# Nahuel-M/StereoVisionArray

Measured on AMD Instinct MI355X. Metric: Mdisparities/sec (W·H·D/s) at 1080p D=128, higher is better.
Workload: dtype u16

## Files before the change

stereovisionarray_amd/csrc/sva_tuning.h:

```cpp
#pragma once

#include <cstddef>

namespace sva {
namespace tune {

constexpr int kPfH4 = 40, kPfV4 = 24;
constexpr int kPfH8 = 32, kPfV8 = 12;
constexpr int kPfH12 = 24, kPfV12 = 8;
constexpr int kPfH16 = 12, kPfV16 = 8;
constexpr int kCLoadAux = 0;
constexpr int kCkptStoreAux = 0;
constexpr int kStaticCkptHitsMaxDpl = 4;

constexpr int kDiagPair4 = 0, kDiagPair8 = 1, kDiagPair12 = 0, kDiagPair16 = 0;
constexpr long long kDiagPairMinPixels = 1450000;
constexpr int kPathMinima4 = 0, kPathMinima8 = 1, kPathMinima12 = 0, kPathMinima16 = 0;
constexpr int kWtahvPfVolPair = 4;
constexpr int kWtahvTileLog2 = 3;
constexpr int kWtahvTileLog2Wide = 3;
constexpr int kWtahvPfVol = 3;
constexpr int kWtahvPfVol4 = 4;
constexpr int kWtahvPfVol16 = 2;
constexpr int kWtahvPinRowMin = 1;
constexpr int kWtahvPinWta = 1;
constexpr int kWtahvMinWaves = 1;

constexpr int kBatchMaxPairs = 8;
constexpr int kBatchCostStreams = 3;
constexpr int kBatchSubFrames = 4;
constexpr size_t kBatchMaxBytes = (size_t)24 << 30;

constexpr int kPlacementTrials = 6;
constexpr size_t kPlacementMinBytes = (size_t)4 << 30;

constexpr int kCensusRows = 16;
constexpr int kCensusCostMinD = 64;
constexpr int kCensusCostRows = 8;
constexpr int kCensusCostRowsSmall = 4;
constexpr int kCensusCostMinGroups = 1536;
constexpr int kCensusCostPx4 = 64, kCensusCostPx8 = 64, kCensusCostPx12 = 64, kCensusCostPx16 = 128;
constexpr int kCostStoreNT = 1;
constexpr int kCensusCostSlotOrder = 1;
constexpr int kCensusCost2Lines = 8;

constexpr int kPlaneOuKB = 24;
constexpr int kPlaneWords = 1024;
constexpr int kPlaneMinBlocks = 3;
constexpr int kPlaneStageMajor = 2;
constexpr int kPlaneNoHoistDiv = 0;
constexpr int kPlanePoLds = 1;
constexpr int kPlaneSplitMin = 3;
constexpr int kPlaneSplitMax = 6;
constexpr int kPlaneSplitRounds = 4;
constexpr int kPlaneSplitInner = 2;
constexpr int kPlaneWalkRange = 1;

}
}
```

stereovisionarray_amd/csrc/wta_hv.hip:

```cpp
#include "sgm_common.h"
#include "wta_common.h"
#include "sva_tuning.h"

namespace sva {
namespace {

using namespace sgm;

constexpr int TB = 256;
constexpr int TW = 16;

struct WtaHvGeom {
    int W, H, D, P1, P2, dmin;
    int ntx, nty;
    int nsx;
    int dreal;
    unsigned vol;
    unsigned hck;
    unsigned vck;
    int tiles;
};

template <int DPL, bool PAIR> constexpr int pf_vol() {
    return PAIR ? tune::kWtahvPfVolPair : DPL >= 16 ? tune::kWtahvPfVol16 : DPL <= 4 ? tune::kWtahvPfVol4 : tune::kWtahvPfVol;
}

#define SVA_WTAHV_CONF 0
#include "wta_hv_tile.inc"
#undef SVA_WTAHV_CONF
#define SVA_WTAHV_CONF 1
#include "wta_hv_tile.inc"
#undef SVA_WTAHV_CONF

template <int DPL, int TYL, bool PAIR, bool MN>
void wtahv_launch_mn(bool pad, dim3 grid, hipStream_t s, hipEvent_t start, hipEvent_t stop,
                     const uint8_t* C, const uint8_t* L4, const uint8_t* CK, const uint8_t* CKV,
                     const uint8_t* MNP, const WtaHvGeom& g, uint16_t* disp, float* sub,
                     const ConfOut* cf) {
    if (cf) {
        if (pad)
            hipExtLaunchKernelGGL((wta_hv_conf_kernel<DPL, TYL, true, PAIR, MN>), grid, dim3(TB), 0,
                                  s, start, stop, 0, C, L4, CK, CKV, MNP, g, disp, sub, *cf);
        else
            hipExtLaunchKernelGGL((wta_hv_conf_kernel<DPL, TYL, false, PAIR, MN>), grid, dim3(TB), 0,
                                  s, start, stop, 0, C, L4, CK, CKV, MNP, g, disp, sub, *cf);
        return;
    }
    if (pad)
        hipExtLaunchKernelGGL((wta_hv_kernel<DPL, TYL, true, PAIR, MN>), grid, dim3(TB), 0, s, start,
                              stop, 0, C, L4, CK, CKV, MNP, g, disp, sub);
    else
        hipExtLaunchKernelGGL((wta_hv_kernel<DPL, TYL, false, PAIR, MN>), grid, dim3(TB), 0, s, start,
                              stop, 0, C, L4, CK, CKV, MNP, g, disp, sub);
}
template <int DPL, int TYL, bool PAIR, bool MNEN>
void wtahv_launch(bool pad, dim3 grid, hipStream_t s, hipEvent_t start, hipEvent_t stop,
                  const uint8_t* C, const uint8_t* L4, const uint8_t* CK, const uint8_t* CKV,
                  const uint8_t* MNP, const WtaHvGeom& g, uint16_t* disp, float* sub,
                  const ConfOut* cf) {
    if constexpr (MNEN) {
        if (MNP) {
            wtahv_launch_mn<DPL, TYL, PAIR, true>(pad, grid, s, start, stop, C, L4, CK, CKV, MNP, g,
                                                  disp, sub, cf);
            return;
        }
    }
    wtahv_launch_mn<DPL, TYL, PAIR, false>(pad, grid, s, start, stop, C, L4, CK, CKV, nullptr, g,
                                           disp, sub, cf);
}

}

bool wta_hv_supported(int D) { return D == 64 || D == 128 || D == 192 || D == 256; }

hipError_t launch_wta_hv(Ctx& c, const uint8_t* C, const uint8_t* L4, const uint8_t* CK,
                         const uint8_t* CKV, int W, int H, int D, int P1, int P2, int dmin,
                         uint16_t* disp, float* sub, int dreal, int npair, bool pair,
                         const uint8_t* MN, const ConfOut* cf) {
    DispatchTimer t(c, "wta_hv");
    if (!wta_hv_supported(D)) return hipErrorInvalidValue;
    const TileGeom tg = tile_geom(W, H, D);
    WtaHvGeom g;
    g.W = W; g.H = H; g.D = D; g.P1 = P1; g.P2 = P2; g.dmin = dmin;
    g.dreal = dreal > 0 && dreal < D ? dreal : D;
    g.ntx = tg.ntx;
    g.nty = tg.nty;
    g.nsx = tg.nsx;
    const size_t vol = (size_t)W * H * D;
    if (vol >= (size_t)1 << 32) return hipErrorInvalidValue;
    g.vol = (unsigned)vol;
    g.hck = (unsigned)(tg.hck_bytes / 2);
    g.vck = (unsigned)(tg.vck_bytes / 2);
    const bool pad = g.dreal < D;
    if (npair < 1) return hipErrorInvalidValue;
    if (cf && (cf->uniqueness < 0 || cf->uniqueness > 100)) return hipErrorInvalidValue;
    g.tiles = g.ntx * g.nty;
    const dim3 grid((unsigned)(g.tiles * npair));
#define SVA_WTAHV(DPL_, TYL_, MN_)                                                            \
    wtahv_launch<DPL_, TYL_, false, (MN_) != 0>(pad, grid, c.stream, t.start, t.stop, C, L4,  \
                                                CK, CKV, MN, g, disp, sub, cf);               \
    t.used = true
#define SVA_WTAHV_P(DPL_, TYL_, EN_, MN_)                                                     \
    if (pair) {                                                                               \
        wtahv_launch<DPL_, TYL_, (EN_) != 0, (MN_) != 0>(pad, grid, c.stream, t.start,        \
                                                         t.stop, C, L4, CK, CKV, MN, g, disp, \
                                                         sub, cf);                            \
        t.used = true;                                                                        \
    } else {                                                                                  \
        SVA_WTAHV(DPL_, TYL_, MN_);                                                           \
    }
    constexpr int TYL = tune::kWtahvTileLog2, TYLW = tune::kWtahvTileLog2Wide;
    if (tg.seg_log2 != (D <= 128 ? TYL : TYLW)) return hipErrorInvalidValue;
    if (pair && (npair != 1 || !diag_pair_ok(D, P2))) return hipErrorInvalidValue;
    if (MN && (npair != 1 || !path_minima_enabled(D) || (1 << tg.seg_log2) != sgm::kMinimaSeg))
        return hipErrorInvalidValue;
    switch (D) {
        case 64: SVA_WTAHV_P(4, TYL, tune::kDiagPair4, tune::kPathMinima4); break;
        case 128: SVA_WTAHV_P(8, TYL, tune::kDiagPair8, tune::kPathMinima8); break;
        case 192: SVA_WTAHV_P(12, TYLW, tune::kDiagPair12, tune::kPathMinima12); break;
        case 256: SVA_WTAHV_P(16, TYLW, tune::kDiagPair16, tune::kPathMinima16); break;
        default: return hipErrorInvalidValue;
    }
#undef SVA_WTAHV_P
#undef SVA_WTAHV
    return hipGetLastError();
}

}
```

stereovisionarray_amd/csrc/wta_hv_tile.inc:

```
template <int DPL, int TYL, bool PAD, bool PAIR, bool MN>
#if SVA_WTAHV_CONF
__global__ __launch_bounds__(TB, tune::kWtahvMinWaves) void wta_hv_conf_kernel(
    const uint8_t* __restrict__ C, const uint8_t* __restrict__ L4, const uint8_t* __restrict__ CK,
    const uint8_t* __restrict__ CKV, const uint8_t* __restrict__ MNP, WtaHvGeom g,
    uint16_t* __restrict__ disp, float* __restrict__ sub, ConfOut cf) {
#else
__global__ __launch_bounds__(TB, tune::kWtahvMinWaves) void wta_hv_kernel(const uint8_t* __restrict__ C,
                                                    const uint8_t* __restrict__ L4,
                                                    const uint8_t* __restrict__ CK,
                                                    const uint8_t* __restrict__ CKV,
                                                    const uint8_t* __restrict__ MNP, WtaHvGeom g,
                                                    uint16_t* __restrict__ disp,
                                                    float* __restrict__ sub) {
#endif
    constexpr int NW = DPL / 4, NP = DPL / 2;
    constexpr int TY = 1 << TYL;
    constexpr int kPfVol = pf_vol<DPL, PAIR>();
    constexpr bool PIN = tune::kWtahvPinRowMin != 0;

    constexpr int SPR = TW / TY;
    static_assert(TY <= TW && TW % TY == 0, "tile rows must divide 16");
    const unsigned f = blockIdx.x / (unsigned)g.tiles;
    const unsigned tb = blockIdx.x - f * (unsigned)g.tiles;
    const int tx = (int)(tb % (unsigned)g.ntx);
    const int ty = (int)(tb / (unsigned)g.ntx);
    constexpr int NV = PAIR ? 2 : 4;
    static_assert(!MN || TY == kMinimaSeg, "path minima: 8-pixel segments");
    C += (size_t)f * g.vol;
    L4 += (size_t)f * NV * g.vol;
    CK += (size_t)f * 2 * g.hck;
    CKV += (size_t)f * 2 * g.vck;
    disp += (size_t)f * (size_t)g.W * (size_t)g.H;
    if (sub) sub += (size_t)f * (size_t)g.W * (size_t)g.H;
#if SVA_WTAHV_CONF
    if (cf.cost_min) cf.cost_min += (size_t)f * (size_t)g.W * (size_t)g.H;
    if (cf.cost_second) cf.cost_second += (size_t)f * (size_t)g.W * (size_t)g.H;
#endif
    const int slot = (int)(threadIdx.x >> 4);
    const int k = (int)(threadIdx.x & 15);
    const int W = g.W, H = g.H;
    const unsigned uD = (unsigned)g.D, uW = (unsigned)W;
    const unsigned P1 = (unsigned)g.P1, P2 = (unsigned)g.P2;
    const int x0 = tx * TW, y0 = ty * TY;
    const int nx = W - x0 < TW ? W - x0 : TW;
    const int ny = H - y0 < TY ? H - y0 : TY;
    const unsigned lane_d = (unsigned)(k * DPL);
    const rsrc_t rC = make_rsrc(C, g.vol);
    unsigned padm[NP];
#pragma unroll
    for (int j = 0; j < NP; j++) {
        const int dl = k * DPL + pair_d<DPL>(j, 0), dh = k * DPL + pair_d<DPL>(j, 1);
        padm[j] = PAD ? ((dl >= g.dreal ? 0x0000ffffu : 0u) | (dh >= g.dreal ? 0xffff0000u : 0u))
                      : 0u;
    }

    __shared__ unsigned vsum[TY * TW * 16 * NP];
    const int vb0 = k * NP, vb1 = k * NP + 4;
    auto vw = [&](int p) -> int { return (p < 4 ? vb0 : vb1) + (p & 3); };

    const bool vcol = slot < nx;
    const int hr = slot / SPR, hseg = slot % SPR;
    const int hx = x0 + hseg * TY;
    const int nh = W - hx < TY ? W - hx : TY;
    const bool hrow = hr < ny && nh > 0;
    const unsigned xv = (unsigned)(x0 + slot), yh = (unsigned)(y0 + hr);

    Words<NW> cv[TY], ch[TY];
#pragma unroll
    for (int r = 0; r < TY; r++)
        cv[r] = bload<NW>(rC, ((unsigned)(y0 + r) * uW + xv) * uD + lane_d);
    auto load_row = [&]() {
#pragma unroll
        for (int j = 0; j < TY; j++)
            ch[j] = bload<NW>(rC, (yh * uW + (unsigned)(hx + j)) * uD + lane_d);
    };
    load_row();
    Words<2> mv[2] = {}, mh[2] = {};
    if constexpr (MN) {
        const unsigned hmn = (unsigned)H * (unsigned)g.nsx * (unsigned)kMinimaSeg;
        const unsigned vmn = (unsigned)g.nty * uW * (unsigned)kMinimaSeg;
        const unsigned vo = ((unsigned)ty * uW + xv) * (unsigned)kMinimaSeg;
        const unsigned ho = ((unsigned)(y0 + (slot / SPR)) * (unsigned)g.nsx +
                             (unsigned)((x0 + (slot % SPR) * TY) >> TYL)) * (unsigned)kMinimaSeg;
#pragma unroll
        for (int d = 0; d < 2; d++) {
            mv[d] = bload<2>(make_rsrc(MNP + 2 * (size_t)hmn + (size_t)d * vmn, vmn), vo);
            mh[d] = bload<2>(make_rsrc(MNP + (size_t)d * hmn, hmn), ho);
        }
    }
    auto given_m = [](unsigned& m, const Words<2>& w, int i) {
        if constexpr (MN) m = minima_byte(w, i);
    };

    auto zero_state = [](unsigned (&A)[NP], unsigned& m) {
#pragma unroll
        for (int j = 0; j < NP; j++) A[j] = 0u;
        m = 0u;
    };
    unsigned Aa[NP], Ab[NP], ma, mb;
    Edges ea, eb;
    if (vcol) {
        if (ty > 0)
            load_state<DPL, PAD, PIN, MN>(make_rsrc(CKV, g.vck), ((unsigned)(ty - 1) * uW + xv) * uD + lane_d,
                                 Aa, ma, padm);
        else
            zero_state(Aa, ma);
        if (y0 + TY < H)
            load_state<DPL, PAD, PIN, MN>(make_rsrc(CKV + g.vck, g.vck),
                                 ((unsigned)(ty + 1) * uW + xv) * uD + lane_d, Ab, mb, padm);
        else
            zero_state(Ab, mb);
        auto keep = [&](unsigned (&dst)[NP], const unsigned (&A)[NP]) {
#pragma unroll
            for (int q = 0; q < NP; q++) dst[q] = A[q];
        };
        auto put_v = [&](int r, const unsigned (&ld)[NP], const unsigned (&Au)[NP],
                         const unsigned (&cw)[NW]) {
            unsigned V[NP];
#pragma unroll
            for (int p = 0; p < NP; p++) V[p] = ld[p] + Au[p];
            if constexpr (PAIR) {
                unsigned c4[NP];
                words_to_pairs<DPL>(cw, c4);
#pragma unroll
                for (int p = 0; p < NP; p++) V[p] += c4[p] << 2;
            }
            unsigned* dst = &vsum[(r * TW + slot) * 16 * NP];
#pragma unroll
            for (int p = 0; p < NP; p++) dst[vw(p)] = V[p];
        };
        unsigned LD[TY][NP];
        for_seq<TY>([&](auto I) {
            constexpr int i = decltype(I)::value;
            unsigned ow[NW];
            if (i < ny) {
                given_m(ma, mv[0], i);
                sgm_step<DPL, PIN, MN>(cv[i].w, Aa, ma, ow, P1, P2, ea);
                keep(LD[i], Aa);
            }
        });
        for_seq<TY>([&](auto Q) {
            constexpr int r = TY - 1 - decltype(Q)::value;
            if (r < ny) {
                unsigned lu[NW];
                given_m(mb, mv[1], TY - 1 - r);
                sgm_step<DPL, PIN, MN>(cv[r].w, Ab, mb, lu, P1, P2, eb);
                put_v(r, LD[r], Ab, cv[r].w);
            }
        });
    }
    const int hs = hx >> TYL;
    const unsigned ckrow = yh * (unsigned)g.nsx;
    Words<NW> ckw[2];
    rsrc_t rV[NV];
#pragma unroll
    for (int r = 0; r < NV; r++) rV[r] = make_rsrc(L4 + (size_t)r * g.vol, g.vol);
    Words<NW> rv[kPfVol][NV];
    auto issue = [&](int s, int j) {
        const unsigned off = (yh * uW + (unsigned)(hx + j)) * uD + lane_d;
#pragma unroll
        for (int r = 0; r < NV; r++) rv[s][r] = bload<NW, 2>(rV[r], off);
    };
    auto issue_first = [&]() {
        ckw[0] = bload<NW>(make_rsrc(CK, g.hck), (ckrow + (unsigned)(hs - 1)) * uD + lane_d);
        ckw[1] = bload<NW>(make_rsrc(CK + g.hck, g.hck), (ckrow + (unsigned)(hs + 1)) * uD + lane_d);
#pragma unroll
        for (int q = 0; q < kPfVol && q < TY; q++) issue(q, TY - 1 - q);
    };
    if (hrow) issue_first();
    __syncthreads();

    if (!hrow) return;
    if (hs > 0) state_from_words<DPL, PAD, PIN, MN>(ckw[0], Aa, ma, padm);
    else zero_state(Aa, ma);
    unsigned LF[TY][NP];
    for_seq<TY>([&](auto I) {
        constexpr int i = decltype(I)::value;
        unsigned ow[NW];
        if (i < nh) {
            given_m(ma, mh[0], i);
            sgm_step<DPL, PIN, MN>(ch[i].w, Aa, ma, ow, P1, P2, ea);
#pragma unroll
            for (int q = 0; q < NP; q++) LF[i][q] = Aa[q];
        }
    });
    if (hx + TY < W) state_from_words<DPL, PAD, PIN, MN>(ckw[1], Aa, ma, padm);
    else zero_state(Aa, ma);
    unsigned dres = 0u, sm = 0u, s0 = 0u;
#if SVA_WTAHV_CONF
    unsigned s2 = 0xffffu;
#endif
    const bool want_sub = sub != nullptr;
    unsigned dpair[NP];
#pragma unroll
    for (int j = 0; j < NP; j++)
        dpair[j] = (lane_d + (unsigned)pair_d<DPL>(j, 0)) | ((lane_d + (unsigned)pair_d<DPL>(j, 1)) << 16);
    unsigned* const vrow = &vsum[(hr * TW + hseg * TY) * 16 * NP];
    for_seq<TY>([&](auto Q) {
        constexpr int q = decltype(Q)::value, j = TY - 1 - q, s = q % kPfVol;
        if (j < nh) {
            unsigned ow[NW];
            given_m(ma, mh[1], q);
            sgm_step<DPL, PIN, MN>(ch[j].w, Aa, ma, ow, P1, P2, ea);
            unsigned* const vpix = vrow + j * 16 * NP;
            unsigned S[NP];
#pragma unroll
            for (int p = 0; p < NP; p++) S[p] = vpix[vw(p)] + Aa[p];
#pragma unroll
            for (int p = 0; p < NP; p++) S[p] += LF[j][p];
#pragma unroll
            for (int r = 0; r < NV; r++) unpack_add<NW>(rv[s][r].w, S);
            if constexpr (PAD) {
#pragma unroll
                for (int p = 0; p < NP; p++) S[p] |= padm[p];
            }
            const unsigned best = wta_pick_key_perm<DPL, PIN && tune::kWtahvPinWta>(S, dpair);
            const int ds = (int)(best & 0xffffu);
            if (want_sub) {
#pragma unroll
                for (int p = 0; p < NP; p++) vpix[vw(p)] = S[p];
            }
            dres = k == j ? (unsigned)ds : dres;
            s0 = k == j ? best >> 16 : s0;
#if SVA_WTAHV_CONF
            const unsigned sec = wta_second_key_perm<DPL, PIN && tune::kWtahvPinWta>(
                S, dpair, (unsigned)ds, lane_d);
            s2 = k == j ? sec : s2;
#endif
        }
        if constexpr (q + kPfVol < TY) {
            __builtin_amdgcn_sched_barrier(0);
            issue(s, TY - 1 - (q + kPfVol));
            __builtin_amdgcn_sched_barrier(0);
        }
    });
    if (want_sub) {
        __builtin_amdgcn_fence(__ATOMIC_RELEASE, "wavefront");
        __builtin_amdgcn_wave_barrier();
        __builtin_amdgcn_fence(__ATOMIC_ACQUIRE, "wavefront");
        if (k < nh) {
            const uint16_t* s16 = reinterpret_cast<const uint16_t*>(vrow + k * 16 * NP);
            const int ds = (int)dres;
            const int dm = ds > 0 ? ds - 1 : 0, dp = ds + 1 < 16 * DPL ? ds + 1 : ds;
            auto at = [&](int d) {
                const int kk = d / DPL, pp = pair_of<DPL>(d % DPL), hh = half_of<DPL>(d % DPL);
                return (unsigned)s16[2 * (kk * NP + pp) + hh];
            };
            sm = at(dm) | (at(dp) << 16);
        }
    }
    if (k < nh) {
        const size_t at = (size_t)yh * (size_t)W + (size_t)(hx + k);
#if SVA_WTAHV_CONF
        if (cf.cost_min) cf.cost_min[at] = (uint16_t)s0;
        if (cf.cost_second) cf.cost_second[at] = (uint16_t)s2;
        const bool rej = conf_reject(s0, s2, cf.uniqueness);
        disp[at] = rej ? (uint16_t)cf.invalid : (uint16_t)(g.dmin + (int)dres);
        if (want_sub) {
            const float v = subpixel(g.dmin, (int)dres, g.dreal, sm & 0xffffu, s0, sm >> 16);
            sub[at] = rej ? __builtin_nanf("") : v;
        }
#else
        disp[at] = (uint16_t)(g.dmin + (int)dres);
        if (want_sub) sub[at] = subpixel(g.dmin, (int)dres, g.dreal, sm & 0xffffu, s0, sm >> 16);
#endif
    }
}
```

Baseline: 335,600.

## Split WTA-HV tile start to overlap horizontal loads with vertical SGM pass

For the pair+minima variant, the horizontal-row cost loads, minima loads, horizontal checkpoint loads and the first volume prefetches are deferred. They are now issued between the forward and backward vertical SGM sweeps rather than upfront. The vertical checkpoint loads are issued together before being decoded. The aim is to cut register pressure and overlap global-memory latency with vertical-pass compute. The risk is that the loads land later, leaving less slack before the horizontal pass, and that the changed live ranges alter the register count.

Result: no change. 338,900, median of 6 (+1.0%).

```diff
diff --git a/stereovisionarray_amd/csrc/sva_tuning.h b/stereovisionarray_amd/csrc/sva_tuning.h
--- a/stereovisionarray_amd/csrc/sva_tuning.h
+++ b/stereovisionarray_amd/csrc/sva_tuning.h
@@ -17,6 +17,8 @@
 constexpr long long kDiagPairMinPixels = 1450000;
 constexpr int kPathMinima4 = 0, kPathMinima8 = 1, kPathMinima12 = 0, kPathMinima16 = 0;
 constexpr int kWtahvPfVolPair = 4;
+constexpr int kWtahvSplitStart = 1;
+constexpr int kWtahvPfVolPairEarly = 4;
 constexpr int kWtahvTileLog2 = 3;
 constexpr int kWtahvTileLog2Wide = 3;
 constexpr int kWtahvPfVol = 3;
diff --git a/stereovisionarray_amd/csrc/wta_hv.hip b/stereovisionarray_amd/csrc/wta_hv.hip
--- a/stereovisionarray_amd/csrc/wta_hv.hip
+++ b/stereovisionarray_amd/csrc/wta_hv.hip
@@ -23,6 +23,10 @@
 
 template <int DPL, bool PAIR> constexpr int pf_vol() {
     return PAIR ? tune::kWtahvPfVolPair : DPL >= 16 ? tune::kWtahvPfVol16 : DPL <= 4 ? tune::kWtahvPfVol4 : tune::kWtahvPfVol;
+}
+
+template <bool PAIR, int PF> constexpr int pf_vol_early() {
+    return !PAIR ? 0 : tune::kWtahvPfVolPairEarly < PF ? tune::kWtahvPfVolPairEarly : PF;
 }
 
 #define SVA_WTAHV_CONF 0
diff --git a/stereovisionarray_amd/csrc/wta_hv_tile.inc b/stereovisionarray_amd/csrc/wta_hv_tile.inc
--- a/stereovisionarray_amd/csrc/wta_hv_tile.inc
+++ b/stereovisionarray_amd/csrc/wta_hv_tile.inc
@@ -17,6 +17,8 @@
     constexpr int TY = 1 << TYL;
     constexpr int kPfVol = pf_vol<DPL, PAIR>();
     constexpr bool PIN = tune::kWtahvPinRowMin != 0;
+    constexpr bool SO = MN && PAIR && tune::kWtahvSplitStart != 0;
+    constexpr int kPfEarly = SO ? pf_vol_early<PAIR, kPfVol < TY ? kPfVol : TY>() : 0;
 
     constexpr int SPR = TW / TY;
     static_assert(TY <= TW && TW % TY == 0, "tile rows must divide 16");
@@ -74,7 +76,7 @@
         for (int j = 0; j < TY; j++)
             ch[j] = bload<NW>(rC, (yh * uW + (unsigned)(hx + j)) * uD + lane_d);
     };
-    load_row();
+    if constexpr (!SO) load_row();
     Words<2> mv[2] = {}, mh[2] = {};
     if constexpr (MN) {
         const unsigned hmn = (unsigned)H * (unsigned)g.nsx * (unsigned)kMinimaSeg;
@@ -85,7 +87,7 @@
 #pragma unroll
         for (int d = 0; d < 2; d++) {
             mv[d] = bload<2>(make_rsrc(MNP + 2 * (size_t)hmn + (size_t)d * vmn, vmn), vo);
-            mh[d] = bload<2>(make_rsrc(MNP + (size_t)d * hmn, hmn), ho);
+            if constexpr (!SO) mh[d] = bload<2>(make_rsrc(MNP + (size_t)d * hmn, hmn), ho);
         }
     }
     auto given_m = [](unsigned& m, const Words<2>& w, int i) {
@@ -96,10 +98,50 @@
 #pragma unroll
         for (int j = 0; j < NP; j++) A[j] = 0u;
         m = 0u;
+    };
+    Words<NW> rv[kPfVol][NV];
+    auto issue_early = [&]() {
+        if constexpr (kPfEarly > 0) {
+            if (hrow) {
+#pragma unroll
+                for (int q = 0; q < kPfEarly; q++) {
+                    const unsigned off = (yh * uW + (unsigned)(hx + TY - 1 - q)) * uD + lane_d;
+#pragma unroll
+                    for (int r = 0; r < NV; r++)
+                        rv[q][r] = bload<NW, 2>(make_rsrc(L4 + (size_t)r * g.vol, g.vol), off);
+                }
+            }
+        }
+    };
+    Words<NW> ckw[2];
+    auto load_h = [&]() {
+        load_row();
+        const unsigned hmn = (unsigned)H * (unsigned)g.nsx * (unsigned)kMinimaSeg;
+        const unsigned hseg0 = yh * (unsigned)g.nsx + (unsigned)(hx >> TYL);
+#pragma unroll
+        for (int d = 0; d < 2; d++)
+            mh[d] = bload<2>(make_rsrc(MNP + (size_t)d * hmn, hmn), hseg0 * (unsigned)kMinimaSeg);
+        if (hrow) {
+            ckw[0] = bload<NW>(make_rsrc(CK, g.hck), (hseg0 - 1u) * uD + lane_d);
+            ckw[1] = bload<NW>(make_rsrc(CK + g.hck, g.hck), (hseg0 + 1u) * uD + lane_d);
+        }
+        issue_early();
     };
     unsigned Aa[NP], Ab[NP], ma, mb;
     Edges ea, eb;
     if (vcol) {
+        if constexpr (SO) {
+            Words<NW> wa = {}, wb = {};
+            if (ty > 0)
+                wa = bload<NW>(make_rsrc(CKV, g.vck), ((unsigned)(ty - 1) * uW + xv) * uD + lane_d);
+            if (y0 + TY < H)
+                wb = bload<NW>(make_rsrc(CKV + g.vck, g.vck),
+                               ((unsigned)(ty + 1) * uW + xv) * uD + lane_d);
+            if (ty > 0) state_from_words<DPL, PAD, PIN, MN>(wa, Aa, ma, padm);
+            else zero_state(Aa, ma);
+            if (y0 + TY < H) state_from_words<DPL, PAD, PIN, MN>(wb, Ab, mb, padm);
+            else zero_state(Ab, mb);
+        } else {
         if (ty > 0)
             load_state<DPL, PAD, PIN, MN>(make_rsrc(CKV, g.vck), ((unsigned)(ty - 1) * uW + xv) * uD + lane_d,
                                  Aa, ma, padm);
@@ -110,6 +152,7 @@
                                  ((unsigned)(ty + 1) * uW + xv) * uD + lane_d, Ab, mb, padm);
         else
             zero_state(Ab, mb);
+        }
         auto keep = [&](unsigned (&dst)[NP], const unsigned (&A)[NP]) {
 #pragma unroll
             for (int q = 0; q < NP; q++) dst[q] = A[q];
@@ -139,6 +182,7 @@
                 keep(LD[i], Aa);
             }
         });
+        if constexpr (SO) load_h();
         for_seq<TY>([&](auto Q) {
             constexpr int r = TY - 1 - decltype(Q)::value;
             if (r < ny) {
@@ -148,24 +192,26 @@
                 put_v(r, LD[r], Ab, cv[r].w);
             }
         });
+    } else {
+        if constexpr (SO) load_h();
     }
     const int hs = hx >> TYL;
     const unsigned ckrow = yh * (unsigned)g.nsx;
-    Words<NW> ckw[2];
     rsrc_t rV[NV];
 #pragma unroll
     for (int r = 0; r < NV; r++) rV[r] = make_rsrc(L4 + (size_t)r * g.vol, g.vol);
-    Words<NW> rv[kPfVol][NV];
     auto issue = [&](int s, int j) {
         const unsigned off = (yh * uW + (unsigned)(hx + j)) * uD + lane_d;
 #pragma unroll
         for (int r = 0; r < NV; r++) rv[s][r] = bload<NW, 2>(rV[r], off);
     };
     auto issue_first = [&]() {
+        if constexpr (!SO) {
         ckw[0] = bload<NW>(make_rsrc(CK, g.hck), (ckrow + (unsigned)(hs - 1)) * uD + lane_d);
         ckw[1] = bload<NW>(make_rsrc(CK + g.hck, g.hck), (ckrow + (unsigned)(hs + 1)) * uD + lane_d);
-#pragma unroll
-        for (int q = 0; q < kPfVol && q < TY; q++) issue(q, TY - 1 - q);
+        }
+#pragma unroll
+        for (int q = kPfEarly; q < kPfVol && q < TY; q++) issue(q, TY - 1 - q);
     };
     if (hrow) issue_first();
     __syncthreads();
```
